# cgranerob/Land-Surface-Temperature-Super-Resolution-with-a-Scale-Invariance-Free-Neural-Approach

Measured on AMD Instinct MI355X. Metric: LST+NDVI 256x256 patches/sec (train fwd+bwd), whole job, higher is better.
Workload: dtype f32; 1 GPU; ModelB SIF-NN-SR2 (gradFTM loss) batch 64/GPU, synthetic 256x256, 1x MI355X, fwd+loss+bwd+Adam; batch_per_gpu=64, patch=256x256 (LST 64x64 + NDVI 256x256), parallelism=dp1, loss=sr2

## Files before the change

land-surface-temperature-super-resolution-with-a-scale-invariance-free-neural-approach_amd/csrc/edge_conv.h:

```cpp
#pragma once
#include "common.h"

int conv_in_fwd_blocks(int B, int H, int W);
int launch_conv_in_fwd(const float* x, const float* w, float* y, float* partials, int B, int H, int W, hipStream_t s);
int launch_conv_in_wgrad(const float* x, const float* dy, float* partials, int nblk, float* dw, int B, int H, int W, hipStream_t s);
int launch_conv_out_fwd(const float* y, const float* scale, const float* shift, const float* w, const float* bias,
                        float* out, int B, int H, int W, hipStream_t s);
int launch_conv_out_dgrad(const float* dsr, const float* w, float* g, int B, int H, int W, hipStream_t s);
int launch_conv_out_wgrad(const float* y, const float* scale, const float* shift, const float* dsr, float* partials,
                          int nblk, float* dw, float* db, int B, int H, int W, hipStream_t s);
int launch_conv_in_wgrad_fused(const float* x, const float* g, const float* y, const float* scale, const float* shift,
                               const double* coef, float* partials, int nblk, float* dw, int B, int H, int W, hipStream_t s);
size_t conv_in_gram_scratch_floats();
int launch_conv_in_gram(const float* x, float* scratch, int B, int H, int W, hipStream_t s);
const double* conv_in_gram_result(const float* scratch);
int launch_conv_in_dz_wgrad(const float* x, const float* dz, float* partials, int nblk, int B, int H, int W, hipStream_t s);
int launch_conv_in_dw_combine(const float* partials, int nblk, const double* gram, const float* w, const double* coef, float* dw,
                              hipStream_t s);
int launch_tail_bwd_reduce(const float* y, const float* scale, const float* shift, const float* mean, const float* invstd,
                           const float* dsr, const float* w, float* wpart, float* bnpart, int nblk, int B, int H, int W,
                           hipStream_t s);
int launch_tail_bwd_apply(const float* y, const float* scale, const float* shift, const double* coef, const float* dsr,
                          const float* w, float* dy, int B, int H, int W, hipStream_t s);
int launch_sum_partials(const float* partials, int nblk, int n, float* out, hipStream_t s);

int launch_bn_finalize(const float* partials, int nblk, int C, double count, const float* gamma, const float* beta,
                       float* run_mean, float* run_var, float momentum, float eps, float* mean, float* invstd,
                       float* scale, float* shift, hipStream_t s);
int launch_bn_eval_coeffs(const float* params, const float* running, float eps, float* scale, float* shift, hipStream_t s);
int launch_bn_bwd_reduce(const float* g, const float* y, const float* scale, const float* shift, const float* mean,
                         const float* invstd, int C, size_t npix, float* partials, int nblk, hipStream_t s,
                         const float* gp = nullptr, int H = 0, int W = 0, float* g_out = nullptr);
int launch_bn_bwd_finalize(const float* partials, int nblk, int C, double count, const float* scale, const float* mean,
                           const float* invstd, float* dgamma, float* dbeta, double* coef, hipStream_t s,
                           const float* shift = nullptr, const float* beta = nullptr, float* coef_f = nullptr,
                           const float* xs_partials = nullptr, int xs_n = 0, float* xs_out = nullptr,
                           int frozen = 0);
int launch_bn_bwd_finalize2(const float* pa, int na, const float* pb, int nb, int C, double count, const float* scale,
                            const float* mean, const float* invstd, float* dgamma, float* dbeta, double* coef, hipStream_t s,
                            const float* shift = nullptr, const float* beta = nullptr, float* coef_f = nullptr, int frozen = 0);
int launch_bn_bwd_apply(const float* g, const float* y, const float* scale, const float* shift, const double* coef,
                        int C, size_t npix, float* dy, hipStream_t s, const float* gp = nullptr, int H = 0, int W = 0);
int launch_nbt_increment(long long* nbt, int n, hipStream_t s);

int launch_bn_frozen_stats(const float* running, float eps, float* mean, float* invstd, hipStream_t s);
int launch_conv_in_dgrad(const float* g, const float* y, const float* scale, const float* shift, const double* coef, const float* w,
                         float* dx, int B, int H, int W, hipStream_t s);

int launch_bnrelu_pool2(const float* y, const float* scale, const float* shift, float* out, int B, int H, int W, int C, hipStream_t s);
int launch_bnrelu_add(const float* p, const float* y, const float* scale, const float* shift, float* out, int C, size_t npix, hipStream_t s);
int launch_bnrelu_up2x(const float* y, const float* scale, const float* shift, float* out, int B, int Hin, int Win, int C, hipStream_t s);
int launch_pool2_bwd(const float* gp, float* g, int B, int H, int W, int C, int accumulate, hipStream_t s);
int launch_up2x_bwd(const float* gu, float* g, int B, int Hin, int Win, int C, hipStream_t s, const float* bn_y = nullptr,
                    const float* bn_scale = nullptr, const float* bn_shift = nullptr, float* bn_partials = nullptr);
int up2x_bwd_stat_rows(int B, int Hin, int Win, int C);

int launch_adam_flat(float* p, const float* g, float* m, float* v, int n, float lr, float beta1, float beta2, float eps,
                     float weight_decay, int step, float grad_scale, hipStream_t s);

int launch_adam_flat_dev(float* p, const float* g, float* m, float* v, int n, float lr, float beta1, float beta2, float eps,
                         float weight_decay, long long* step_dev, float* coef2, float grad_scale, hipStream_t s);

int launch_tiles_prepare(const float* lst, const float* ndvi, float* x, int T, int tiles_x, int win, long long lst_step_y,
                         long long lst_step_x, int lst_row, long long ndvi_step_y, long long ndvi_step_x, int ndvi_row,
                         float mean_lst, float std_lst, float mean_ndvi, float std_ndvi, int clip_ndvi, hipStream_t s);
int launch_tiles_paste(const float* sr, float* out, int T, int tiles_x, int hr, long long out_row, float mean, float std,
                       hipStream_t s);
int launch_l4pool4(const float* x, float* out, int B, int H, int W, hipStream_t s);
size_t psnr_ssim_scratch_bytes(int B, int H, int W);
int launch_psnr_ssim(const float* pred, const float* targ, int B, int H, int W, void* scratch, float* out2, hipStream_t s);
size_t psnr_ssim_masked_scratch_bytes(int B, int H, int W);
int launch_psnr_ssim_masked(const float* pred, const float* targ, const unsigned char* valid, int scale, int B, int H, int W,
                            void* scratch, float* out2, int* counts2, hipStream_t s);

size_t eval_metrics_scratch_bytes(int B, int H, int W);
int launch_eval_metrics(const float* a, const float* b, int B, int H, int W, const float* taps9, float data_range,
                        void* scratch, double* out8, hipStream_t s);
int launch_gradient_strata(const float* a, int B, int H, int W, const float* taps9, float* g, float* q2, int* counts3,
                           hipStream_t s);
size_t eval_metrics_masked_scratch_bytes(int B, int H, int W);
int launch_eval_metrics_masked(const float* a, const float* b, const unsigned char* mask, int B, int H, int W,
                               const float* taps9, float data_range, void* scratch, double* out8, int* counts5, hipStream_t s);

size_t fourier_scratch_bytes(int B, int H, int W);
int launch_fft2_attenuation(const float* img, int B, int H, int W, void* scratch, float* mag, float* spectrum, hipStream_t s);
```

land-surface-temperature-super-resolution-with-a-scale-invariance-free-neural-approach_amd/csrc/edge_conv.hip:

```cpp
#include "edge_conv.h"

namespace {

template <bool HS>
__global__ __launch_bounds__(256) void conv_in_fwd_kernel(const float* __restrict__ x, const float* __restrict__ w,
                                                          float* __restrict__ y, float* __restrict__ partials,
                                                          int B, int H, int W) {
  __shared__ float tile[2][2 * 324];
  __shared__ float red[4][16][2];
  const int tid = threadIdx.x, lane = tid & 63, wave = tid >> 6;
  const int i = lane & 15, kq = lane >> 4;
  const int tiles_x = (W + 15) / 16, tiles_y = (H + 15) / 16, ntiles = B * tiles_x * tiles_y;
  auto stage = [&](int t, float* dst) {
    const int tx = t % tiles_x, ty = (t / tiles_x) % tiles_y, b = t / (tiles_x * tiles_y);
    const int x0 = tx * 16, y0 = ty * 16;
    for (int e = tid; e < 2 * 324; e += 256) {
      const int c = e / 324, p = e - c * 324;
      const int py = p / 18, px = p - py * 18;
      const int gy = clampi(y0 - 1 + py, 0, H - 1), gx = clampi(x0 - 1 + px, 0, W - 1);
      dst[e] = x[((size_t)(b * 2 + c) * H + gy) * W + gx];
    }
  };
  if ((int)blockIdx.x < ntiles) stage(blockIdx.x, tile[0]);
  float wa[5];
  int off[5];
#pragma unroll
  for (int j = 0; j < 5; ++j) {
    const int kk = 4 * j + kq;
    wa[j] = kk < 18 ? w[i * 18 + kk] : 0.f;
    const int c = kk >= 9 ? 1 : 0, t = kk < 18 ? kk - 9 * c : 0;
    off[j] = (kk < 18 ? c * 324 : 0) + (t / 3) * 18 + t % 3 + i;
  }
  float s1[4] = {0.f, 0.f, 0.f, 0.f}, s2[4] = {0.f, 0.f, 0.f, 0.f};
  int buf = 0;
  for (int t = blockIdx.x; t < ntiles; t += gridDim.x, buf ^= 1) {
    __syncthreads();
    if (t + (int)gridDim.x < ntiles) stage(t + gridDim.x, tile[buf ^ 1]);
    const int tx = t % tiles_x, ty = (t / tiles_x) % tiles_y, b = t / (tiles_x * tiles_y);
    const int x0 = tx * 16, y0 = ty * 16;
    const float* T = tile[buf];
#pragma unroll
    for (int r = 0; r < 4; ++r) {
      const int row = 4 * wave + r;
      f32x4 acc = (f32x4){0.f, 0.f, 0.f, 0.f};
#pragma unroll
      for (int j = 0; j < 5; ++j) acc = __builtin_amdgcn_mfma_f32_16x16x4f32(wa[j], T[off[j] + row * 18], acc, 0, 0, 0);
      if (y0 + row < H && x0 + i < W) {
        const float4 o = as_stored4<HS>(make_float4(acc[0], acc[1], acc[2], acc[3]));
        stA4<HS>(y, ((size_t)(b * H + y0 + row) * W + x0 + i) * 16 + 4 * kq, o);
        const float ov[4] = {o.x, o.y, o.z, o.w};
#pragma unroll
        for (int q = 0; q < 4; ++q) { s1[q] += ov[q]; s2[q] = fmaf(ov[q], ov[q], s2[q]); }
      }
    }
  }
  if (partials != nullptr) {
#pragma unroll
    for (int q = 0; q < 4; ++q) {
#pragma unroll
      for (int m = 1; m < 16; m <<= 1) { s1[q] += __shfl_xor(s1[q], m); s2[q] += __shfl_xor(s2[q], m); }
      if (i == 0) { red[wave][4 * kq + q][0] = s1[q]; red[wave][4 * kq + q][1] = s2[q]; }
    }
    __syncthreads();
    if (tid < 32) {
      const int co = tid >> 1, j = tid & 1;
      const float s = red[0][co][j] + red[1][co][j] + red[2][co][j] + red[3][co][j];
      partials[((size_t)blockIdx.x * 16 + co) * 2 + j] = s;
    }
  }
}

template <bool FUSED, bool HS>
__global__ __launch_bounds__(256) void conv_in_wgrad_kernel(const float* __restrict__ x, const float* __restrict__ dy,
                                                            const float* __restrict__ yraw,
                                                            const float* __restrict__ scale,
                                                            const float* __restrict__ shift,
                                                            const double* __restrict__ coef,
                                                            float* __restrict__ partials, int B, int H, int W) {
  SIFSR_CHAIN_PRIO();
  __shared__ float tile[2 * 324 + 8];
  __shared__ float dyt[256 * 16];
  __shared__ float red[4][2][256];
  const int tid = threadIdx.x, lane = tid & 63, wave = tid >> 6;
  const int tiles_x = (W + 15) / 16, tiles_y = (H + 15) / 16, ntiles = B * tiles_x * tiles_y;
  const int i16 = lane & 15, k = lane >> 4;
  int offn[2];
#pragma unroll
  for (int nt = 0; nt < 2; ++nt) {
    const int n = nt * 16 + i16;
    offn[nt] = n < 18 ? (n / 9) * 324 + ((n % 9) / 3) * 18 + (n % 9) % 3 : 0;
  }
  f32x4 acc[2] = {(f32x4){0.f, 0.f, 0.f, 0.f}, (f32x4){0.f, 0.f, 0.f, 0.f}};
  float4 sc4, sh4;
  double sd[4], k1[4], k0[4];
  if (FUSED) {
    const int q4 = tid & 3;
    sc4 = ld4(scale + 4 * q4); sh4 = ld4(shift + 4 * q4);
#pragma unroll
    for (int j = 0; j < 4; ++j) { sd[j] = coef[4 * q4 + j]; k1[j] = coef[16 + 4 * q4 + j]; k0[j] = coef[32 + 4 * q4 + j]; }
  }
  for (int tl = blockIdx.x; tl < ntiles; tl += gridDim.x) {
    const int tx = tl % tiles_x, ty = (tl / tiles_x) % tiles_y, b = tl / (tiles_x * tiles_y);
    const int x0 = tx * 16, y0 = ty * 16;
    __syncthreads();
    for (int e = tid; e < 2 * 324; e += 256) {
      const int c = e / 324, p = e - c * 324;
      const int py = p / 18, px = p - py * 18;
      const int gy = clampi(y0 - 1 + py, 0, H - 1), gx = clampi(x0 - 1 + px, 0, W - 1);
      tile[e] = x[((size_t)(b * 2 + c) * H + gy) * W + gx];
    }
    for (int e = tid; e < 256 * 4; e += 256) {
      const int p = e >> 2, c4 = e & 3;
      if (y0 + (p >> 4) >= H || x0 + (p & 15) >= W) {
        *reinterpret_cast<float4*>(&dyt[p * 16 + 4 * c4]) = make_float4(0.f, 0.f, 0.f, 0.f);
        continue;
      }
      const size_t off = ((size_t)(b * H + y0 + (p >> 4)) * W + x0 + (p & 15)) * 16 + 4 * c4;
      float4 v = ldA4<HS>(dy, off);
      if (FUSED) {
        const float4 yv = ldA4<HS>(yraw, off);
        v.x = (float)fma(sd[0], (double)(fmaf(yv.x, sc4.x, sh4.x) > 0.f ? v.x : 0.f), fma(k1[0], (double)yv.x, k0[0]));
        v.y = (float)fma(sd[1], (double)(fmaf(yv.y, sc4.y, sh4.y) > 0.f ? v.y : 0.f), fma(k1[1], (double)yv.y, k0[1]));
        v.z = (float)fma(sd[2], (double)(fmaf(yv.z, sc4.z, sh4.z) > 0.f ? v.z : 0.f), fma(k1[2], (double)yv.z, k0[2]));
        v.w = (float)fma(sd[3], (double)(fmaf(yv.w, sc4.w, sh4.w) > 0.f ? v.w : 0.f), fma(k1[3], (double)yv.w, k0[3]));
      }
      *reinterpret_cast<float4*>(&dyt[p * 16 + 4 * c4]) = v;
    }
    __syncthreads();
#pragma unroll 4
    for (int ks = wave; ks < 64; ks += 4) {
      const int r = ks >> 2, qd = ks & 3;
      const float av = dyt[(r * 16 + 4 * qd + k) * 16 + i16];
      const int base = r * 18 + 4 * qd + k;
      acc[0] = __builtin_amdgcn_mfma_f32_16x16x4f32(av, tile[offn[0] + base], acc[0], 0, 0, 0);
      acc[1] = __builtin_amdgcn_mfma_f32_16x16x4f32(av, tile[offn[1] + base], acc[1], 0, 0, 0);
    }
  }
#pragma unroll
  for (int nt = 0; nt < 2; ++nt)
#pragma unroll
    for (int r = 0; r < 4; ++r) red[wave][nt][(4 * k + r) * 16 + i16] = acc[nt][r];
  __syncthreads();
  for (int e = tid; e < 288; e += 256) {
    const int co = e / 18, n = e % 18;
    const int nt = n >> 4, col = n & 15;
    partials[(size_t)blockIdx.x * 288 + e] =
        red[0][nt][co * 16 + col] + red[1][nt][co * 16 + col] + red[2][nt][co * 16 + col] + red[3][nt][co * 16 + col];
  }
}

constexpr int OCS = 20;

template <bool HS>
__global__ __launch_bounds__(256) void conv_out_fwd_kernel(const float* __restrict__ y, const float* scale,
                                                           const float* shift, const float* __restrict__ w,
                                                           const float* __restrict__ bias, float* __restrict__ out,
                                                           int H, int W) {
  constexpr int NGRP = 21;
  __shared__ float P[NGRP * 16 * 9];
  const int tid = threadIdx.x, lane = tid & 63, wave = tid >> 6;
  const int i = lane & 15, kq = lane >> 4;
  const int x0 = blockIdx.x * 16, y0 = blockIdx.y * 16, b = blockIdx.z;
  float wb[4];
#pragma unroll
  for (int j = 0; j < 4; ++j) wb[j] = i < 9 ? w[(4 * kq + j) * 9 + i] : 0.f;
  float4 sc = make_float4(1.f, 1.f, 1.f, 1.f), sh = make_float4(0.f, 0.f, 0.f, 0.f);
  if (scale != nullptr) { sc = ld4(scale + 4 * kq); sh = ld4(shift + 4 * kq); }
  constexpr int NPW = (NGRP + 3) / 4;
  float4 v[NPW];
#pragma unroll
  for (int n = 0; n < NPW; ++n) {
    const int g = wave + 4 * n;
    int p = g * 16 + i;
    if (p > 323) p = 323;
    const int r = p / 18, c = p - r * 18;
    const int gy = clampi(y0 - 1 + r, 0, H - 1), gx = clampi(x0 - 1 + c, 0, W - 1);
    v[n] = ldA4<HS>(y, ((size_t)(b * H + gy) * W + gx) * 16 + 4 * kq);
  }
#pragma unroll
  for (int n = 0; n < NPW; ++n) {
    const int g = wave + 4 * n;
    if (g >= NGRP) break;
    float4 a = v[n];
    if (scale != nullptr) a = bn_relu4(a, sc, sh);
    f32x4 acc = (f32x4){0.f, 0.f, 0.f, 0.f};
    acc = __builtin_amdgcn_mfma_f32_16x16x4f32(a.x, wb[0], acc, 0, 0, 0);
    acc = __builtin_amdgcn_mfma_f32_16x16x4f32(a.y, wb[1], acc, 0, 0, 0);
    acc = __builtin_amdgcn_mfma_f32_16x16x4f32(a.z, wb[2], acc, 0, 0, 0);
    acc = __builtin_amdgcn_mfma_f32_16x16x4f32(a.w, wb[3], acc, 0, 0, 0);
    if (i < 9) {
#pragma unroll
      for (int r = 0; r < 4; ++r) P[(g * 16 + 4 * kq + r) * 9 + i] = acc[r];
    }
  }
  __syncthreads();
  const int ty = tid >> 4, tx = tid & 15;
  float s = bias[0];
#pragma unroll
  for (int t = 0; t < 9; ++t) s += P[((ty + t / 3) * 18 + tx + t % 3) * 9 + t];
  if (y0 + ty < H && x0 + tx < W) out[(size_t)(b * H + y0 + ty) * W + x0 + tx] = s;
}

template <bool HS>
__global__ __launch_bounds__(256) void conv_out_dgrad_kernel(const float* __restrict__ dsr, const float* __restrict__ w,
                                                             float* __restrict__ g, int B, int H, int W) {
  const size_t n = (size_t)B * H * W;
  for (size_t q = (size_t)blockIdx.x * blockDim.x + threadIdx.x; q < n; q += (size_t)gridDim.x * blockDim.x) {
    const int qx = q % W, qy = (q / W) % H;
    const size_t img = q - (size_t)qy * W - qx;
    float S[9];
#pragma unroll
    for (int t = 0; t < 9; ++t) {
      const int ty = t / 3 - 1, tx = t % 3 - 1;
      int ys[2], ny = 0, xs[2], nx = 0;
      if (qy - ty >= 0 && qy - ty < H) ys[ny++] = qy - ty;
      if ((qy == 0 && ty == -1) || (qy == H - 1 && ty == 1)) ys[ny++] = qy;
      if (qx - tx >= 0 && qx - tx < W) xs[nx++] = qx - tx;
      if ((qx == 0 && tx == -1) || (qx == W - 1 && tx == 1)) xs[nx++] = qx;
      float s = 0.f;
      for (int iy = 0; iy < ny; ++iy)
        for (int ix = 0; ix < nx; ++ix) s += dsr[img + (size_t)ys[iy] * W + xs[ix]];
      S[t] = s;
    }
#pragma unroll
    for (int c4 = 0; c4 < 4; ++c4) {
      float o[4];
#pragma unroll
      for (int j = 0; j < 4; ++j) {
        float s = 0.f;
#pragma unroll
        for (int t = 0; t < 9; ++t) s = fmaf(w[(4 * c4 + j) * 9 + t], S[t], s);
        o[j] = s;
      }
      stA4<HS>(g, q * 16 + 4 * c4, make_float4(o[0], o[1], o[2], o[3]));
    }
  }
}

template <bool HS>
__global__ __launch_bounds__(256) void conv_out_wgrad_kernel(const float* __restrict__ y, const float* scale,
                                                             const float* shift, const float* __restrict__ dsr,
                                                             float* __restrict__ partials, int B, int H, int W) {
  __shared__ float tile[18 * 20 * OCS];
  __shared__ float dt[256];
  __shared__ float red[4][256];
  __shared__ float bsum[4];
  const int tid = threadIdx.x, lane = tid & 63, wave = tid >> 6;
  const int tiles_x = (W + 15) / 16, tiles_y = (H + 15) / 16, ntiles = B * tiles_x * tiles_y;
  const int i16 = lane & 15, k = lane >> 4;
  const int tty = i16 < 9 ? i16 / 3 : 100, ttx = i16 < 9 ? i16 % 3 : 100;
  f32x4 acc = (f32x4){0.f, 0.f, 0.f, 0.f};
  float bacc = 0.f;
  for (int e = tid; e < 18 * 20 * OCS; e += 256) tile[e] = 0.f;
  for (int tl = blockIdx.x; tl < ntiles; tl += gridDim.x) {
    const int tx = tl % tiles_x, ty = (tl / tiles_x) % tiles_y, b = tl / (tiles_x * tiles_y);
    const int x0 = tx * 16, y0 = ty * 16;
    __syncthreads();
    for (int e = tid; e < 324 * 4; e += 256) {
      const int p = e >> 2, c4 = e & 3;
      const int py = p / 18, px = p - py * 18;
      const int gy = clampi(y0 - 1 + py, 0, H - 1), gx = clampi(x0 - 1 + px, 0, W - 1);
      float4 v = ldA4<HS>(y, ((size_t)(b * H + gy) * W + gx) * 16 + 4 * c4);
      if (scale != nullptr) v = bn_relu4(v, ld4(scale + 4 * c4), ld4(shift + 4 * c4));
      *reinterpret_cast<float4*>(&tile[(py * 20 + px) * OCS + 4 * c4]) = v;
// ... 138 lines not shown
                                                                  float* __restrict__ partials, int B, int H, int W) {
  SIFSR_CHAIN_PRIO();
  __shared__ float tile[2][2 * 324 + 8];
  __shared__ float red[4][4][72];
  const int tid = threadIdx.x, lane = tid & 63, wave = tid >> 6;
  const int tiles_x = (W + 15) / 16, tiles_y = (H + 15) / 16, ntiles = B * tiles_x * tiles_y;
  const int c4 = tid & 3, pl = tid >> 2;
  const int lx = pl & 15, ly0 = pl >> 4;
  f32x2 acc[4][9];
#pragma unroll
  for (int j = 0; j < 4; ++j)
#pragma unroll
    for (int u = 0; u < 9; ++u) acc[j][u] = (f32x2){0.f, 0.f};
  float4 pz[4];
  float px_[3];
  size_t nbase = 0;
  int nrow[4] = {0, 0, 0, 0};
  bool nin[4] = {false, false, false, false};
  auto fetch_z = [&](int k) __attribute__((always_inline)) { pz[k] = ldA4<HS>(dz, nbase + (size_t)nrow[k]); };
  auto fetch = [&](int tl) __attribute__((always_inline)) {
    const int tx = tl % tiles_x, r = tl / tiles_x, ty = r % tiles_y, b = r / tiles_y;
    const int x0 = tx * 16, y0 = ty * 16;
    const int gx = min(x0 + lx, W - 1);
    nbase = ((size_t)(b * H) * W + gx) * 16 + 4 * c4;
#pragma unroll
    for (int k = 0; k < 4; ++k) {
      nrow[k] = min(y0 + ly0 + 4 * k, H - 1) * W * 16;
      nin[k] = y0 + ly0 + 4 * k < H && x0 + lx < W;
    }
#pragma unroll
    for (int i = 0; i < 3; ++i) {
      const int e = min(tid + 256 * i, 2 * 324 - 1);
      const int c = e / 324, p = e - c * 324;
      const int py = p / 18, pxx = p - py * 18;
      px_[i] = x[((size_t)(b * 2 + c) * H + clampi(y0 - 1 + py, 0, H - 1)) * W + clampi(x0 - 1 + pxx, 0, W - 1)];
    }
  };
  int buf = 0;
  bool cin_[4] = {false, false, false, false};
  if ((int)blockIdx.x < ntiles) {
    fetch(blockIdx.x);
#pragma unroll
    for (int k = 0; k < 4; ++k) fetch_z(k);
  }
  for (int tl = blockIdx.x; tl < ntiles; tl += gridDim.x, buf ^= 1) {
    tile[buf][tid] = px_[0];
    tile[buf][tid + 256] = px_[1];
    if (tid + 512 < 2 * 324) tile[buf][tid + 512] = px_[2];
#pragma unroll
    for (int k = 0; k < 4; ++k) cin_[k] = nin[k];
    __syncthreads();
    fetch(tl + (int)gridDim.x < ntiles ? tl + (int)gridDim.x : tl);
    const float* T = tile[buf];
#pragma unroll
    for (int k = 0; k < 4; ++k) {
      float4 zv = pz[k];
      fetch_z(k);
      __builtin_amdgcn_sched_barrier(0);
      if (!cin_[k]) zv = make_float4(0.f, 0.f, 0.f, 0.f);
      const int ly = ly0 + 4 * k;
      f32x2 pp[9];
#pragma unroll
      for (int u = 0; u < 9; ++u) {
        const int n0 = 2 * u, n1 = 2 * u + 1;
        pp[u] = (f32x2){T[(n0 / 9) * 324 + (ly + (n0 % 9) / 3) * 18 + lx + (n0 % 9) % 3],
                        T[(n1 / 9) * 324 + (ly + (n1 % 9) / 3) * 18 + lx + (n1 % 9) % 3]};
      }
      const float zz[4] = {zv.x, zv.y, zv.z, zv.w};
#pragma unroll
      for (int j = 0; j < 4; ++j)
#pragma unroll
        for (int u = 0; u < 9; ++u) acc[j][u] = __builtin_elementwise_fma((f32x2){zz[j], zz[j]}, pp[u], acc[j][u]);
    }
  }
#pragma unroll
  for (int j = 0; j < 4; ++j)
#pragma unroll
    for (int u = 0; u < 9; ++u)
#pragma unroll
      for (int h = 0; h < 2; ++h) {
        float v = acc[j][u][h];
#pragma unroll
        for (int m = 4; m < 64; m <<= 1) v += __shfl_xor(v, m);
        if (lane < 4) red[wave][c4][j * 18 + 2 * u + h] = v;
      }
  __syncthreads();
  for (int e = tid; e < 288; e += 256) {
    const int co = e / 18, n = e - co * 18;
    const int q = co >> 2, i = (co & 3) * 18 + n;
    partials[(size_t)blockIdx.x * 288 + e] = red[0][q][i] + red[1][q][i] + red[2][q][i] + red[3][q][i];
  }
}

__global__ __launch_bounds__(64) void conv_in_dw_combine_kernel(const float* __restrict__ partials, int nblk,
                                                                const double* __restrict__ gram, const float* __restrict__ w,
                                                                const double* __restrict__ coef, float* __restrict__ dw) {
  const int e = blockIdx.x, lane = threadIdx.x;
  const int c = e / 18, k = e - c * 18;
  double s = 0.0;
  for (int r = lane; r < nblk; r += 64) s += (double)partials[(size_t)r * 288 + e];
#pragma unroll
  for (int m = 32; m > 0; m >>= 1) s += __shfl_xor(s, m);
  if (lane == 0) {
    double a = 0.0;
    for (int kr = 0; kr < 18; ++kr) a += (double)w[c * 18 + kr] * gram[kr <= k ? gram_idx(kr, k) : gram_idx(k, kr)];
    dw[e] = (float)(coef[c] * s + coef[16 + c] * a + coef[32 + c] * gram[171 + k]);
  }
}

__global__ __launch_bounds__(256) void sum_partials_kernel(const float* __restrict__ partials, int nblk, int n,
                                                           float* __restrict__ out) {
  __shared__ double part[64][4];
  const int el = threadIdx.x & 3, grp = threadIdx.x >> 2;
  const int e = blockIdx.x * 4 + el;
  double s = 0.0;
  if (e < n)
    for (int k = grp; k < nblk; k += 64) s += (double)partials[(size_t)k * n + e];
  part[grp][el] = s;
  __syncthreads();
  for (int st = 32; st > 0; st >>= 1) {
    if (grp < st) part[grp][el] += part[grp + st][el];
    __syncthreads();
  }
  if (grp == 0 && e < n) out[e] = (float)part[0][el];
}

}

int conv_in_fwd_blocks(int B, int H, int W) {
  const int ntiles = B * ((H + 15) / 16) * ((W + 15) / 16);
  return ntiles < 2048 ? ntiles : 2048;
}

int launch_conv_in_fwd(const float* x, const float* w, float* y, float* partials, int B, int H, int W, hipStream_t s) {
  if (H < 1 || W < 1 || B < 1) return SIFSR_ERR_SHAPE;
  if (sifsr_half_storage()) hipLaunchKernelGGL(conv_in_fwd_kernel<true>, dim3(conv_in_fwd_blocks(B, H, W)), dim3(256), 0, s, x, w, y, partials, B, H, W);
  else hipLaunchKernelGGL(conv_in_fwd_kernel<false>, dim3(conv_in_fwd_blocks(B, H, W)), dim3(256), 0, s, x, w, y, partials, B, H, W);
  SIFSR_LAUNCH_CHECK();
  return SIFSR_OK;
}

int launch_conv_in_wgrad(const float* x, const float* dy, float* partials, int nblk, float* dw, int B, int H, int W,
                         hipStream_t s) {
  if (H < 1 || W < 1) return SIFSR_ERR_SHAPE;
  if (sifsr_half_storage()) hipLaunchKernelGGL((conv_in_wgrad_kernel<false, true>), dim3(nblk), dim3(256), 0, s, x, dy, nullptr, nullptr, nullptr, nullptr, partials, B, H, W);
  else hipLaunchKernelGGL((conv_in_wgrad_kernel<false, false>), dim3(nblk), dim3(256), 0, s, x, dy, nullptr, nullptr, nullptr, nullptr, partials, B, H, W);
  hipLaunchKernelGGL(sum_partials_kernel, dim3(72), dim3(256), 0, s, partials, nblk, 288, dw);
  SIFSR_LAUNCH_CHECK();
  return SIFSR_OK;
}

int launch_conv_in_wgrad_fused(const float* x, const float* g, const float* y, const float* scale, const float* shift,
                               const double* coef, float* partials, int nblk, float* dw, int B, int H, int W,
                               hipStream_t s) {
  if (H < 1 || W < 1) return SIFSR_ERR_SHAPE;
  if (sifsr_half_storage()) hipLaunchKernelGGL((conv_in_wgrad_kernel<true, true>), dim3(nblk), dim3(256), 0, s, x, g, y, scale, shift, coef, partials, B, H, W);
  else hipLaunchKernelGGL((conv_in_wgrad_kernel<true, false>), dim3(nblk), dim3(256), 0, s, x, g, y, scale, shift, coef, partials, B, H, W);
  hipLaunchKernelGGL(sum_partials_kernel, dim3(72), dim3(256), 0, s, partials, nblk, 288, dw);
  SIFSR_LAUNCH_CHECK();
  return SIFSR_OK;
}

size_t conv_in_gram_scratch_floats() { return (size_t)1024 * GRAM_PITCH + 2 * GRAM_PITCH; }
int launch_conv_in_gram(const float* x, float* scratch, int B, int H, int W, hipStream_t s) {
  if (H < 1 || W < 1 || B < 1) return SIFSR_ERR_SHAPE;
  const int ntiles = B * ((H + 15) / 16) * ((W + 15) / 16);
  const int nblk = ntiles < 512 ? ntiles : 512;
  if (H % 16 == 0 && W % 16 == 0) hipLaunchKernelGGL(conv_in_gram_kernel<true>, dim3(nblk), dim3(256), 0, s, x, scratch, B, H, W);
  else hipLaunchKernelGGL(conv_in_gram_kernel<false>, dim3(nblk), dim3(256), 0, s, x, scratch, B, H, W);
  hipLaunchKernelGGL(conv_in_gram_reduce_kernel, dim3(GRAM_N), dim3(64), 0, s, scratch, nblk, reinterpret_cast<double*>(scratch + (size_t)1024 * GRAM_PITCH));
  SIFSR_LAUNCH_CHECK();
  return SIFSR_OK;
}
const double* conv_in_gram_result(const float* scratch) { return reinterpret_cast<const double*>(scratch + (size_t)1024 * GRAM_PITCH); }

int launch_conv_in_dz_wgrad(const float* x, const float* dz, float* partials, int nblk, int B, int H, int W, hipStream_t s) {
  if (H < 1 || W < 1 || nblk < 1) return SIFSR_ERR_SHAPE;
  if (sifsr_half_storage()) hipLaunchKernelGGL(conv_in_dz_wgrad_kernel<true>, dim3(nblk), dim3(256), 0, s, x, dz, partials, B, H, W);
  else hipLaunchKernelGGL(conv_in_dz_wgrad_kernel<false>, dim3(nblk), dim3(256), 0, s, x, dz, partials, B, H, W);
  SIFSR_LAUNCH_CHECK();
  return SIFSR_OK;
}
int launch_conv_in_dw_combine(const float* partials, int nblk, const double* gram, const float* w, const double* coef, float* dw,
                              hipStream_t s) {
  hipLaunchKernelGGL(conv_in_dw_combine_kernel, dim3(288), dim3(64), 0, s, partials, nblk, gram, w, coef, dw);
  SIFSR_LAUNCH_CHECK();
  return SIFSR_OK;
}

int launch_conv_out_fwd(const float* y, const float* scale, const float* shift, const float* w, const float* bias,
                        float* out, int B, int H, int W, hipStream_t s) {
  if (H < 1 || W < 1) return SIFSR_ERR_SHAPE;
  if (sifsr_half_storage()) hipLaunchKernelGGL(conv_out_fwd_kernel<true>, dim3((W + 15) / 16, (H + 15) / 16, B), dim3(256), 0, s, y, scale, shift, w, bias, out, H, W);
  else hipLaunchKernelGGL(conv_out_fwd_kernel<false>, dim3((W + 15) / 16, (H + 15) / 16, B), dim3(256), 0, s, y, scale, shift, w, bias, out, H, W);
  SIFSR_LAUNCH_CHECK();
  return SIFSR_OK;
}

int launch_conv_out_dgrad(const float* dsr, const float* w, float* g, int B, int H, int W, hipStream_t s) {
  const size_t n = (size_t)B * H * W;
  int blocks = (int)((n + 255) / 256);
  if (blocks > 8192) blocks = 8192;
  if (sifsr_half_storage()) hipLaunchKernelGGL(conv_out_dgrad_kernel<true>, dim3(blocks), dim3(256), 0, s, dsr, w, g, B, H, W);
  else hipLaunchKernelGGL(conv_out_dgrad_kernel<false>, dim3(blocks), dim3(256), 0, s, dsr, w, g, B, H, W);
  SIFSR_LAUNCH_CHECK();
  return SIFSR_OK;
}

int launch_conv_out_wgrad(const float* y, const float* scale, const float* shift, const float* dsr, float* partials,
                          int nblk, float* dw, float* db, int B, int H, int W, hipStream_t s) {
  if (H < 1 || W < 1) return SIFSR_ERR_SHAPE;
  if (sifsr_half_storage()) hipLaunchKernelGGL(conv_out_wgrad_kernel<true>, dim3(nblk), dim3(256), 0, s, y, scale, shift, dsr, partials, B, H, W);
  else hipLaunchKernelGGL(conv_out_wgrad_kernel<false>, dim3(nblk), dim3(256), 0, s, y, scale, shift, dsr, partials, B, H, W);
  if (db != dw + 144) return SIFSR_ERR_ARG;
  hipLaunchKernelGGL(sum_partials_kernel, dim3(37), dim3(256), 0, s, partials, nblk, 145, dw);
  SIFSR_LAUNCH_CHECK();
  return SIFSR_OK;
}

int launch_sum_partials(const float* partials, int nblk, int n, float* out, hipStream_t s) {
  hipLaunchKernelGGL(sum_partials_kernel, dim3((n + 3) / 4), dim3(256), 0, s, partials, nblk, n, out);
  SIFSR_LAUNCH_CHECK();
  return SIFSR_OK;
}
```

land-surface-temperature-super-resolution-with-a-scale-invariance-free-neural-approach_amd/csrc/engine.hip:

```cpp
#include "engine.h"
#include "switches.h"

#include <stdio.h>
#include <stdlib.h>

#include <mutex>
#include <vector>

static thread_local bool t_half_storage = false;
bool sifsr_half_storage() { return t_half_storage; }
HalfStorageScope::HalfStorageScope(bool on) : prev(t_half_storage) { t_half_storage = on; }
HalfStorageScope::~HalfStorageScope() { t_half_storage = prev; }

static int env_int(const char* name, int dflt) { const char* v = getenv(name); return v ? atoi(v) : dflt; }
const Switches& sifsr_switches() {
  static const Switches sw = {
      env_int("SIFSR_WGRAD_STREAM", 1), env_int("SIFSR_WGRAD_WINO", 2),  env_int("SIFSR_NO_WINO", 0),
      env_int("SIFSR_NO_WINO8", 0),     env_int("SIFSR_NO_BWD16", 0),    env_int("SIFSR_TAIL_APPLY", 0),
      env_int("SIFSR_HEAD_LINEAR", 0),  env_int("SIFSR_BF16_BWD16", 0),  env_int("SIFSR_DBG_EARLY_REDUCE", 3),
      env_int("SIFSR_DBG_POOL_ON_LOAD", 1)};
  return sw;
}

static constexpr int enc_prev[3] = {L_IN3, L_D1C, L_D2C};
// ... 463 lines not shown
    SIFSR_TRY(launch_bn_eval_coeffs(params, running, eps, c.f(w.scale), c.f(w.shift), s));
  }

  SIFSR_TRY(launch_conv_in_fwd(x, params + nt.L[L_IN0].w_off, c.y(L_IN0), training ? c.f(w.partials) : nullptr, B, H, W, s));
  if (training) SIFSR_TRY(bn_unit_finalize(c, L_IN0, conv_in_fwd_blocks(B, H, W), running, momentum, eps));
  SIFSR_TRY(conv_unit_fwd(c, L_IN3, src_act(c, L_IN0), src_none(), training, running, momentum, eps));

  for (int k = 0; k < 3; ++k) {
    const int lp = enc_prev[k];
    SIFSR_TRY(launch_bnrelu_pool2(c.y(lp), c.scale(lp), c.shift(lp), c.f(w.P[k]), B, c.lvH(k), c.lvW(k), pc[k], s));
    SIFSR_TRY(conv_unit_fwd(c, enc_a[k], src_raw(c.f(w.P[k]), pc[k]), src_none(), training, running, momentum, eps));
    SIFSR_TRY(conv_unit_fwd(c, enc_b[k], src_act(c, enc_a[k]), src_none(), training, running, momentum, eps));
    SIFSR_TRY(launch_bnrelu_add(c.f(w.P[k]), c.y(enc_b[k]), c.scale(enc_b[k]), c.shift(enc_b[k]), c.f(w.R[k]), pc[k],
                                w.npix[k + 1], s));
    SIFSR_TRY(conv_unit_fwd(c, enc_c[k], src_raw(c.f(w.R[k]), pc[k]), src_none(), training, running, momentum, eps));
  }

  for (int k = 0; k < 3; ++k) {
    const int lv = 2 - k;
    const int ll = dec_low[k];
    SIFSR_TRY(launch_bnrelu_up2x(c.y(ll), c.scale(ll), c.shift(ll), c.f(w.U[k]), B, c.lvH(lv + 1), c.lvW(lv + 1), uc[k], s));
    SIFSR_TRY(conv_unit_fwd(c, dec_a[k], src_raw(c.f(w.U[k]), uc[k]), src_act(c, dec_skip[k]), training, running, momentum, eps));
    SIFSR_TRY(conv_unit_fwd(c, dec_b[k], src_act(c, dec_a[k]), src_none(), training, running, momentum, eps));
  }

  SIFSR_TRY(launch_conv_out_fwd(c.y(L_U3B), c.scale(L_U3B), c.shift(L_U3B), params + nt.out_w_off,
                                params + nt.out_b_off, sr, B, H, W, s));
  return SIFSR_OK;
}

int sifsr_engine_forward_frozen(const float* x, float* sr, const float* params, const float* running, float* ws, size_t ws_floats,
                                int B, int H, int W, float eps, hipStream_t s) {
  if (!running || !ws) return SIFSR_ERR_ARG;
  WsLayout lay;
  SIFSR_TRY(sifsr_layout(B, H, W, 1, &lay));
  if (ws_floats < lay.total) return SIFSR_ERR_WORKSPACE;
  SIFSR_TRY(sifsr_engine_forward(x, sr, params, const_cast<float*>(running), nullptr, ws, ws_floats, B, H, W, 0, 0.f, eps, s, 0));
  return launch_bn_frozen_stats(running, eps, ws + lay.mean, ws + lay.invstd, s);
}

int sifsr_engine_backward(const float* x, const float* dsr, const float* params, float* grads, float* ws,
                          size_t ws_floats, int B, int H, int W, hipStream_t s, int bf16, int frozen, float* dx) {
  if (!x || !dsr || !params || !grads || !ws) return SIFSR_ERR_ARG;
  Ctx c{sifsr_net(), WsLayout(), ws, params, B, H, W, s};
  if (bf16 < 0 || bf16 > 1) return SIFSR_ERR_ARG;
  if ((frozen != 0 || dx != nullptr) && bf16 != 0) return SIFSR_ERR_ARG;
  c.bf16 = bf16;
  c.frozen = frozen != 0;
  const HalfStorageScope storage(bf16 == 1);
  SIFSR_TRY(sifsr_layout(B, H, W, 1, &c.lay));
  if (ws_floats < c.lay.total) return SIFSR_ERR_WORKSPACE;
  const NetTable& nt = c.nt;
  const WsLayout& w = c.lay;
  const Switches& sw = sifsr_switches();
  BwdState state;
  c.grads = grads; c.bwd = &state;
  c.side = (size_t)B * H * W >= 2u * 65536u || g_side_override == 1 ? side_lane(s) : nullptr;
  SideLaneGuard lane_guard(c.side, s);
  c.forked = &lane_guard.forked;

  const bool head_linear = sw.head_linear != 0 && dx == nullptr && bwd16_usable(c, L_IN3, src_act(c, L_IN0));
  if (head_linear) {
    hipStream_t gs = s;
    if (c.side != nullptr) {
      if (hipEventRecord(c.side->ev[L_IN0], s) != hipSuccess || hipStreamWaitEvent(c.side->s, c.side->ev[L_IN0], 0) != hipSuccess) return SIFSR_ERR_ARG;
      lane_guard.forked = true;
      gs = c.side->s;
    }
    SIFSR_TRY(launch_conv_in_gram(x, c.f(w.gram), B, H, W, gs));
    if (c.side != nullptr && hipEventRecord(c.side->aux, gs) != hipSuccess) return SIFSR_ERR_ARG;
  }
  const bool tail_in_bwd16 = !sw.tail_apply && bwd16_usable(c, L_U3B, src_act(c, L_U3A));
  {
    const LayerInfo& L = nt.L[L_U3B];
    int nblk = B * ((H + 15) / 16) * ((W + 15) / 16);
    if (nblk > 768) nblk = 768;
    SIFSR_TRY(launch_tail_bwd_reduce(c.y(L_U3B), c.scale(L_U3B), c.shift(L_U3B), c.mean(L_U3B), c.invstd(L_U3B), dsr,
                                     params + nt.out_w_off, c.f(w.slabs), c.f(w.partials), nblk, B, H, W, s));
    if (grads + nt.out_b_off != grads + nt.out_w_off + 144) return SIFSR_ERR_ARG;
    SIFSR_TRY(launch_bn_bwd_finalize(c.f(w.partials), nblk, 16, (double)w.npix[0], c.scale(L_U3B), c.mean(L_U3B), c.invstd(L_U3B),
                                     grads + L.gamma_off, grads + L.beta_off, c.coef(), s, c.shift(L_U3B), params + L.beta_off,
                                     c.coef_f(L_U3B), c.f(w.slabs), 145, grads + nt.out_w_off, c.frozen));
    if (!tail_in_bwd16)
      SIFSR_TRY(launch_tail_bwd_apply(c.y(L_U3B), c.scale(L_U3B), c.shift(L_U3B), c.coef(), dsr, params + nt.out_w_off, c.g(L_U3B),
                                      B, H, W, s));
  }

  int up_rows = 0;
  for (int k = 2; k >= 0; --k) {
    const int lv = 2 - k;
    const int la = dec_a[k], lb = dec_b[k], ls = dec_skip[k], ll = dec_low[k];
    if (k != 2) SIFSR_TRY(bn_unit_bwd(c, lb, nullptr, up_rows, 0));
    int rows_a = 0;
    SIFSR_TRY(conv_unit_bwd(c, lb, src_act(c, la), k == 2 && tail_in_bwd16 ? dsr : c.g(lb), c.g(la), nullptr, la, &rows_a,
                            k == 2 ? (tail_in_bwd16 ? 2 : 0) : 1));
    SIFSR_TRY(bn_unit_bwd(c, la, nullptr, rows_a));
    SIFSR_TRY(conv_unit_wgrad(c, la, src_raw(c.f(w.U[k]), uc[k]), src_act(c, ls), c.g(la)));
    SIFSR_TRY(conv_unit_dgrad(c, la, c.g(la), c.f(w.gU[k]), uc[k], uc[k], c.g(ls), nt.L[ls].cout, nullptr));
    up_rows = up2x_bwd_stat_rows(B, c.lvH(lv + 1), c.lvW(lv + 1), uc[k]);
    if ((size_t)up_rows * uc[k] * 2 > w.partials_cap) up_rows = 0;
    SIFSR_TRY(launch_up2x_bwd(c.f(w.gU[k]), c.g(ll), B, c.lvH(lv + 1), c.lvW(lv + 1), uc[k], s,
                              up_rows ? c.y(ll) : nullptr, up_rows ? c.scale(ll) : nullptr, up_rows ? c.shift(ll) : nullptr,
                              up_rows ? c.f(w.partials) : nullptr));
  }

  for (int k = 2; k >= 0; --k) {
    const int la = enc_a[k], lb = enc_b[k], lc = enc_c[k];
    const int er = sw.early_reduce;
    if (c.side != nullptr && (er == 3 || (er == 2 && k != 1) || (er == 1 && k == 0))) SIFSR_TRY(finish_wgrads_side(c));
    SIFSR_TRY(bn_unit_bwd(c, lc, k < 2 ? c.f(w.gP[k + 1]) : nullptr, k == 2 ? up_rows : 0, 0));
    SIFSR_TRY(conv_unit_wgrad(c, lc, src_raw(c.f(w.R[k]), pc[k]), src_none(), c.g(lc)));
    int rows_b = 0, rows_a = 0;
    SIFSR_TRY(conv_unit_dgrad(c, lc, c.g(lc), c.g(lb), pc[k], pc[k], nullptr, 0, nullptr, lb, &rows_b));
    SIFSR_TRY(bn_unit_bwd(c, lb, nullptr, rows_b));
    SIFSR_TRY(conv_unit_bwd(c, lb, src_act(c, la), c.g(lb), c.g(la), nullptr, la, &rows_a));
    SIFSR_TRY(bn_unit_bwd(c, la, nullptr, rows_a));
    SIFSR_TRY(conv_unit_bwd(c, la, src_raw(c.f(w.P[k]), pc[k]), c.g(la), c.f(w.gP[k]), c.g(lb), -1, nullptr));
  }

  const bool pool_on_load = sw.pool_on_load != 0 && bwd16_usable(c, L_IN3, src_act(c, L_IN0));
  SIFSR_TRY(bn_unit_bwd(c, L_IN3, c.f(w.gP[0]), 0, -1, !pool_on_load));
  int rows_in0 = 0;
  bool fused_in3 = false;
  SIFSR_TRY(conv_unit_bwd16(c, L_IN3, src_act(c, L_IN0), c.g(L_IN3), c.g(L_IN0), nullptr, L_IN0, &rows_in0, 1, &fused_in3, head_linear,
                            pool_on_load ? c.f(w.gP[0]) : nullptr));
  if (pool_on_load && !fused_in3) return SIFSR_ERR_ARG;
  if (head_linear && !fused_in3) return SIFSR_ERR_ARG;
  if (!fused_in3) SIFSR_TRY(conv_unit_wgrad(c, L_IN3, src_act(c, L_IN0), src_none(), c.g(L_IN3)));
  if (c.side != nullptr) SIFSR_TRY(finish_wgrads_side(c));
  if (!fused_in3) SIFSR_TRY(conv_unit_dgrad(c, L_IN3, c.g(L_IN3), c.g(L_IN0), 16, 16, nullptr, 0, nullptr, L_IN0, &rows_in0));
  {
    const LayerInfo& L = nt.L[L_IN0];
    if (rows_in0 > 0) {
      SIFSR_TRY(bn_unit_bwd(c, L_IN0, nullptr, rows_in0));
    } else {
      const size_t npix = w.npix[0];
      const int nblk_r = bn_bwd_reduce_blocks(npix);
      SIFSR_TRY(launch_bn_bwd_reduce(c.g(L_IN0), c.y(L_IN0), c.scale(L_IN0), c.shift(L_IN0), c.mean(L_IN0), c.invstd(L_IN0), 16, npix,
                                     c.f(w.partials), nblk_r, s));
      SIFSR_TRY(launch_bn_bwd_finalize(c.f(w.partials), nblk_r, 16, (double)npix, c.scale(L_IN0), c.mean(L_IN0), c.invstd(L_IN0),
                                       grads + L.gamma_off, grads + L.beta_off, c.coef(), s, nullptr, nullptr, nullptr, nullptr, 0, nullptr,
                                       c.frozen));
    }
    int nblk = B * ((H + 15) / 16) * ((W + 15) / 16);
    if (head_linear) {
      if (nblk > 768) nblk = 768;
      SIFSR_TRY(launch_conv_in_dz_wgrad(x, c.g(L_IN0), c.f(w.slabs), nblk, B, H, W, s));
      if (c.side != nullptr && hipStreamWaitEvent(s, c.side->aux, 0) != hipSuccess) return SIFSR_ERR_ARG;
      SIFSR_TRY(launch_conv_in_dw_combine(c.f(w.slabs), nblk, conv_in_gram_result(c.f(w.gram)), params + L.w_off, c.coef(),
                                          grads + L.w_off, s));
    } else {
      if (nblk > 1024) nblk = 1024;
      SIFSR_TRY(launch_conv_in_wgrad_fused(x, c.g(L_IN0), c.y(L_IN0), c.scale(L_IN0), c.shift(L_IN0), c.coef(), c.f(w.slabs), nblk,
                                           grads + L.w_off, B, H, W, s));
    }
    if (dx != nullptr)
      SIFSR_TRY(launch_conv_in_dgrad(c.g(L_IN0), c.y(L_IN0), c.scale(L_IN0), c.shift(L_IN0), c.coef(), params + L.w_off, dx, B, H, W, s));
  }
  if (c.side != nullptr) {
    SIFSR_TRY(lane_guard.join());
  } else {
    SIFSR_TRY(finish_wgrads(c, s));
  }
  return SIFSR_OK;
}

int sifsr_engine_set_wgrad_stream(int on) {
  g_side_override = on < 0 ? -1 : (on ? 1 : 0);
  return SIFSR_OK;
}

static int prof_add_locked(int layer, int phase) {
  if (g_prof.active >= PROF_SLOTS) return -1;
  ProfSlot& p = g_prof.slot[g_prof.active];
  while (p.start.size() < PROF_POOL) {
    hipEvent_t e0, e1;
    if (hipEventCreate(&e0) != hipSuccess) break;
    if (hipEventCreate(&e1) != hipSuccess) { (void)hipEventDestroy(e0); break; }
    p.start.push_back(e0); p.stop.push_back(e1);
  }
  p.used = 0; p.layer = layer; p.phase = phase;
  return g_prof.active++;
}
int sifsr_engine_profile_select(int layer, int phase) {
  std::lock_guard<std::mutex> lk(g_prof.mu);
  g_prof.active = 0;
  if (layer >= 0 && prof_add_locked(layer, phase) < 0) return SIFSR_ERR_ARG;
  return SIFSR_OK;
}
int sifsr_engine_profile_add(int layer, int phase) {
  if (layer < 0) return -1;
  std::lock_guard<std::mutex> lk(g_prof.mu);
  return prof_add_locked(layer, phase);
}
int sifsr_engine_profile_read(int slot, float* total_ms, int* count) {
  std::lock_guard<std::mutex> lk(g_prof.mu);
  float tot = 0.f; int n = 0;
  if (slot >= 0 && slot < g_prof.active) {
    ProfSlot& p = g_prof.slot[slot];
    for (size_t i = 0; i < p.used; ++i) {
      float ms = 0.f;
      if (hipEventSynchronize(p.stop[i]) == hipSuccess && hipEventElapsedTime(&ms, p.start[i], p.stop[i]) == hipSuccess) { tot += ms; ++n; }
    }
  }
  if (total_ms) *total_ms = tot;
  if (count) *count = n;
  return SIFSR_OK;
}
```

Measured before the change: 10730 patches/s.

## Recompute first conv output via MFMA in input-layer wgrad instead of reloading y

The first-layer weight-gradient kernel gains a RECOMP path that rebuilds the raw conv output y from the input tile and the weights with MFMA, so it no longer reads the stored 16-channel y tensor. The path also prefetches the next tile's input pixels and g into registers while the current tile is processed, and the launch bounds now request 4 blocks per CU. The aim is to cut global memory traffic and hide load latency. The cost is extra MFMA work and register pressure, plus a possible rounding difference from the recomputed y.

Measured after the change: 10770 patches/s, median of 6. About the same (+0.4%).

```diff
diff --git a/land-surface-temperature-super-resolution-with-a-scale-invariance-free-neural-approach_amd/csrc/edge_conv.h b/land-surface-temperature-super-resolution-with-a-scale-invariance-free-neural-approach_amd/csrc/edge_conv.h
--- a/land-surface-temperature-super-resolution-with-a-scale-invariance-free-neural-approach_amd/csrc/edge_conv.h
+++ b/land-surface-temperature-super-resolution-with-a-scale-invariance-free-neural-approach_amd/csrc/edge_conv.h
@@ -10,7 +10,8 @@
 int launch_conv_out_wgrad(const float* y, const float* scale, const float* shift, const float* dsr, float* partials,
                           int nblk, float* dw, float* db, int B, int H, int W, hipStream_t s);
 int launch_conv_in_wgrad_fused(const float* x, const float* g, const float* y, const float* scale, const float* shift,
-                               const double* coef, float* partials, int nblk, float* dw, int B, int H, int W, hipStream_t s);
+                               const double* coef, float* partials, int nblk, float* dw, int B, int H, int W, hipStream_t s,
+                               const float* w = nullptr);
 size_t conv_in_gram_scratch_floats();
 int launch_conv_in_gram(const float* x, float* scratch, int B, int H, int W, hipStream_t s);
 const double* conv_in_gram_result(const float* scratch);
diff --git a/land-surface-temperature-super-resolution-with-a-scale-invariance-free-neural-approach_amd/csrc/edge_conv.hip b/land-surface-temperature-super-resolution-with-a-scale-invariance-free-neural-approach_amd/csrc/edge_conv.hip
--- a/land-surface-temperature-super-resolution-with-a-scale-invariance-free-neural-approach_amd/csrc/edge_conv.hip
+++ b/land-surface-temperature-super-resolution-with-a-scale-invariance-free-neural-approach_amd/csrc/edge_conv.hip
@@ -70,13 +70,15 @@
   }
 }
 
-template <bool FUSED, bool HS>
-__global__ __launch_bounds__(256) void conv_in_wgrad_kernel(const float* __restrict__ x, const float* __restrict__ dy,
+template <bool FUSED, bool HS, bool RECOMP = false>
+__global__ __launch_bounds__(256, 4) void conv_in_wgrad_kernel(const float* __restrict__ x, const float* __restrict__ dy,
                                                             const float* __restrict__ yraw,
                                                             const float* __restrict__ scale,
                                                             const float* __restrict__ shift,
                                                             const double* __restrict__ coef,
-                                                            float* __restrict__ partials, int B, int H, int W) {
+                                                            float* __restrict__ partials, int B, int H, int W,
+                                                            const float* __restrict__ w = nullptr) {
+  static_assert(FUSED || !RECOMP, "y is recomputed only to form dy from (g, y)");
   SIFSR_CHAIN_PRIO();
   __shared__ float tile[2 * 324 + 8];
   __shared__ float dyt[256 * 16];
@@ -94,22 +96,77 @@
   float4 sc4, sh4;
   double sd[4], k1[4], k0[4];
   if (FUSED) {
-    const int q4 = tid & 3;
+    const int q4 = RECOMP ? k : tid & 3;
     sc4 = ld4(scale + 4 * q4); sh4 = ld4(shift + 4 * q4);
 #pragma unroll
     for (int j = 0; j < 4; ++j) { sd[j] = coef[4 * q4 + j]; k1[j] = coef[16 + 4 * q4 + j]; k0[j] = coef[32 + 4 * q4 + j]; }
+  }
+  float wa[5];
+  int off[5];
+  float4 pg[4];
+  float pxv[3];
+  auto issue_g = [&](int tl) {
+    const int tx = tl % tiles_x, ty = (tl / tiles_x) % tiles_y, b = tl / (tiles_x * tiles_y);
+    const int x0 = tx * 16, y0 = ty * 16;
+#pragma unroll
+    for (int it = 0; it < 3; ++it) {
+      const int e = tid + 256 * it < 2 * 324 ? tid + 256 * it : 2 * 324 - 1;
+      const int c = e / 324, p = e - c * 324;
+      const int py = p / 18, px = p - py * 18;
+      const int gy = clampi(y0 - 1 + py, 0, H - 1), gx = clampi(x0 - 1 + px, 0, W - 1);
+      pxv[it] = x[((size_t)(b * 2 + c) * H + gy) * W + gx];
+    }
+#pragma unroll
+    for (int r = 0; r < 4; ++r) {
+      const int row = 4 * wave + r;
+      pg[r] = make_float4(0.f, 0.f, 0.f, 0.f);
+      if (y0 + row < H && x0 + i16 < W) pg[r] = ldA4<HS>(dy, ((size_t)(b * H + y0 + row) * W + x0 + i16) * 16 + 4 * k);
+    }
+  };
+  if (RECOMP) {
+#pragma unroll
+    for (int j = 0; j < 5; ++j) {
+      const int kk = 4 * j + k;
+      wa[j] = kk < 18 ? w[i16 * 18 + kk] : 0.f;
+      const int c = kk >= 9 ? 1 : 0, t = kk < 18 ? kk - 9 * c : 0;
+      off[j] = (kk < 18 ? c * 324 : 0) + (t / 3) * 18 + t % 3 + i16;
+    }
+    if ((int)blockIdx.x < ntiles) issue_g(blockIdx.x);
   }
   for (int tl = blockIdx.x; tl < ntiles; tl += gridDim.x) {
     const int tx = tl % tiles_x, ty = (tl / tiles_x) % tiles_y, b = tl / (tiles_x * tiles_y);
     const int x0 = tx * 16, y0 = ty * 16;
     __syncthreads();
-    for (int e = tid; e < 2 * 324; e += 256) {
+    for (int e = tid; !RECOMP && e < 2 * 324; e += 256) {
       const int c = e / 324, p = e - c * 324;
       const int py = p / 18, px = p - py * 18;
       const int gy = clampi(y0 - 1 + py, 0, H - 1), gx = clampi(x0 - 1 + px, 0, W - 1);
       tile[e] = x[((size_t)(b * 2 + c) * H + gy) * W + gx];
     }
-    for (int e = tid; e < 256 * 4; e += 256) {
+    if (RECOMP) {
+#pragma unroll
+      for (int it = 0; it < 3; ++it)
+        if (tid + 256 * it < 2 * 324) tile[tid + 256 * it] = pxv[it];
+      __syncthreads();
+#pragma unroll
+      for (int r = 0; r < 4; ++r) {
+        const int row = 4 * wave + r;
+        f32x4 ya = (f32x4){0.f, 0.f, 0.f, 0.f};
+#pragma unroll
+        for (int j = 0; j < 5; ++j) ya = __builtin_amdgcn_mfma_f32_16x16x4f32(wa[j], tile[off[j] + row * 18], ya, 0, 0, 0);
+        const float4 yv = as_stored4<HS>(make_float4(ya[0], ya[1], ya[2], ya[3]));
+        float4 v = pg[r];
+        if (y0 + row < H && x0 + i16 < W) {
+          v.x = (float)fma(sd[0], (double)(fmaf(yv.x, sc4.x, sh4.x) > 0.f ? v.x : 0.f), fma(k1[0], (double)yv.x, k0[0]));
+          v.y = (float)fma(sd[1], (double)(fmaf(yv.y, sc4.y, sh4.y) > 0.f ? v.y : 0.f), fma(k1[1], (double)yv.y, k0[1]));
+          v.z = (float)fma(sd[2], (double)(fmaf(yv.z, sc4.z, sh4.z) > 0.f ? v.z : 0.f), fma(k1[2], (double)yv.z, k0[2]));
+          v.w = (float)fma(sd[3], (double)(fmaf(yv.w, sc4.w, sh4.w) > 0.f ? v.w : 0.f), fma(k1[3], (double)yv.w, k0[3]));
+        }
+        *reinterpret_cast<float4*>(&dyt[(row * 16 + i16) * 16 + 4 * k]) = v;
+      }
+      if (tl + (int)gridDim.x < ntiles) issue_g(tl + gridDim.x);
+    }
+    for (int e = tid; !RECOMP && e < 256 * 4; e += 256) {
       const int p = e >> 2, c4 = e & 3;
       if (y0 + (p >> 4) >= H || x0 + (p & 15) >= W) {
         *reinterpret_cast<float4*>(&dyt[p * 16 + 4 * c4]) = make_float4(0.f, 0.f, 0.f, 0.f);
@@ -554,8 +611,12 @@
 
 int launch_conv_in_wgrad_fused(const float* x, const float* g, const float* y, const float* scale, const float* shift,
                                const double* coef, float* partials, int nblk, float* dw, int B, int H, int W,
-                               hipStream_t s) {
+                               hipStream_t s, const float* w) {
   if (H < 1 || W < 1) return SIFSR_ERR_SHAPE;
+  if (w != nullptr) {
+    if (sifsr_half_storage()) hipLaunchKernelGGL((conv_in_wgrad_kernel<true, true, true>), dim3(nblk), dim3(256), 0, s, x, g, nullptr, scale, shift, coef, partials, B, H, W, w);
+    else hipLaunchKernelGGL((conv_in_wgrad_kernel<true, false, true>), dim3(nblk), dim3(256), 0, s, x, g, nullptr, scale, shift, coef, partials, B, H, W, w);
+  } else
   if (sifsr_half_storage()) hipLaunchKernelGGL((conv_in_wgrad_kernel<true, true>), dim3(nblk), dim3(256), 0, s, x, g, y, scale, shift, coef, partials, B, H, W);
   else hipLaunchKernelGGL((conv_in_wgrad_kernel<true, false>), dim3(nblk), dim3(256), 0, s, x, g, y, scale, shift, coef, partials, B, H, W);
   hipLaunchKernelGGL(sum_partials_kernel, dim3(72), dim3(256), 0, s, partials, nblk, 288, dw);
diff --git a/land-surface-temperature-super-resolution-with-a-scale-invariance-free-neural-approach_amd/csrc/engine.hip b/land-surface-temperature-super-resolution-with-a-scale-invariance-free-neural-approach_amd/csrc/engine.hip
--- a/land-surface-temperature-super-resolution-with-a-scale-invariance-free-neural-approach_amd/csrc/engine.hip
+++ b/land-surface-temperature-super-resolution-with-a-scale-invariance-free-neural-approach_amd/csrc/engine.hip
@@ -639,7 +639,7 @@
     } else {
       if (nblk > 1024) nblk = 1024;
       SIFSR_TRY(launch_conv_in_wgrad_fused(x, c.g(L_IN0), c.y(L_IN0), c.scale(L_IN0), c.shift(L_IN0), c.coef(), c.f(w.slabs), nblk,
-                                           grads + L.w_off, B, H, W, s));
+                                           grads + L.w_off, B, H, W, s, params + L.w_off));
     }
     if (dx != nullptr)
       SIFSR_TRY(launch_conv_in_dgrad(c.g(L_IN0), c.y(L_IN0), c.scale(L_IN0), c.shift(L_IN0), c.coef(), params + L.w_off, dx, B, H, W, s));
```
